# gildas-lormeau/zlib-streams-ts

Hardware: NVIDIA B200
Metric: deflate_input_GBps (higher is better)
Workload: dtype u8

## Files before the change

### zlib-streams-ts_b200/csrc/zs_lz77.cu

```cuda
#include <cstdio>
#include <cstdlib>

#include "zs_common.cuh"

namespace {

#ifndef ZS_SEARCH_WARPS
#define ZS_SEARCH_WARPS 30
#endif
#ifndef ZS_HASH_BITS
#define ZS_HASH_BITS 14
#endif
#ifndef ZS_LZ_PREV_POS
#define ZS_LZ_PREV_DELTA 1
#endif
constexpr int kSearchWarps = ZS_SEARCH_WARPS;
constexpr int kWarpParse = kSearchWarps;
constexpr int kWarpInsert = kSearchWarps + 1;
constexpr int kThreads = 32 * (kSearchWarps + 2);
constexpr int kStep = 32 * kSearchWarps;
constexpr unsigned kMaxDist = 32768u - 2u * kStep;
constexpr unsigned kNoPrev = 0xffffu;
constexpr unsigned kSymLimit = 16383u;
constexpr unsigned kTooFar = 4096u;
constexpr unsigned kHashBits = ZS_HASH_BITS;
constexpr unsigned kRing = 65536;
constexpr unsigned kRingGuard = 288;
constexpr unsigned pow2_at_least(unsigned v) { unsigned r = 1; while (r < v) r <<= 1; return r; }
constexpr unsigned kResRing = pow2_at_least(4 * kStep + 64);
constexpr unsigned kMjRing = pow2_at_least(3 * kStep + 64);
constexpr unsigned kPbRing = pow2_at_least(2 * kSearchWarps + 4);
constexpr unsigned kMaxSegChunks = 256;

struct LevelCfg { int lazy_fn, good, lazy, nice, chain; };
constexpr LevelCfg kLevels[10] = {
    {0, 0, 0, 0, 0},      {0, 4, 4, 8, 4},      {0, 4, 5, 16, 8},      {0, 4, 6, 32, 32},
    {1, 4, 4, 16, 16},    {1, 8, 16, 32, 32},   {1, 8, 16, 128, 128},  {1, 8, 32, 128, 256},
    {1, 32, 128, 258, 1024}, {1, 32, 258, 258, 4096}};
__host__ __device__ constexpr LevelCfg level_cfg(int level) { return kLevels[level]; }

constexpr uint32_t PREP_HAS_PRED = 1u << 21, PREP_LAST = 1u << 22, PREP_VALID = 1u << 23;

struct Smem {
    uint8_t ring[kRing + kRingGuard];
    uint16_t head[1 << kHashBits];
    uint16_t prev[32768];
    uint32_t prep[3 * kStep];
    uint16_t oldh[2 * kStep];
    uint2 pb[kPbRing];
    uint32_t res[kResRing];
    uint2 mj[kMjRing];
    uint32_t bnd[kMaxSegChunks + 1];
    uint32_t seg;
    uint32_t claim[2];
    alignas(8) uint64_t stage_bar;
};
static_assert(sizeof(Smem) <= 227 * 1024, "shared memory budget");

struct LzArgs {
    const uint8_t* buf;
    uint64_t org;
    uint64_t valid_lo;
    uint64_t data_end;
    const uint64_t* in_off;
    uint32_t n_chunks, seg_chunks, n_seg, max_bpc;
    uint32_t n_big, seg_small;
    LevelCfg cfg;
    int strategy;
    int cross;
    uint32_t* sym;
    uint32_t* chunk_nblk;
    uint32_t* blk_desc;
    uint32_t* seg_counter;
    unsigned stop_after, stop_active;
};

#ifdef ZS_LZ_PROF
__device__ unsigned long long g_prof[16];
#define PROF_T(i) if (lane == 0) atomicAdd(&g_prof[i], (unsigned long long)(clock64() - t_begin))
#else
#define PROF_T(i)
#endif

__device__ __forceinline__ unsigned res_slot(uint32_t q) { return q & (kResRing - 1u); }
__device__ __forceinline__ unsigned mj_slot(uint32_t q) { return q & (kMjRing - 1u); }

__device__ __forceinline__ uint32_t win32(const Smem& S, uint64_t pos) {
    const unsigned idx = (unsigned)pos & (kRing - 1u);
    const unsigned al = idx & ~3u;
    const uint32_t lo = *reinterpret_cast<const uint32_t*>(S.ring + al);
    const uint32_t hi = *reinterpret_cast<const uint32_t*>(S.ring + al + 4);
    return __funnelshift_r(lo, hi, (idx & 3u) * 8u);
}

__device__ __forceinline__ void stage_window(Smem& S, const LzArgs& a, uint64_t from, uint64_t to, unsigned tid, unsigned nthr) {
    const uint64_t safe16 = (a.data_end + 15) & ~15ull;
    for (uint64_t pos = from + 16ull * tid; pos < to; pos += 16ull * nthr) {
        uint4 v = make_uint4(0, 0, 0, 0);
        if (pos < safe16) v = __ldg(reinterpret_cast<const uint4*>(a.buf + pos));
        const unsigned idx = (unsigned)pos & (kRing - 1u);
        *reinterpret_cast<uint4*>(S.ring + idx) = v;
        if (idx < kRingGuard) *reinterpret_cast<uint4*>(S.ring + kRing + idx) = v;
    }
}

#ifndef ZS_LZ_NO_BULK
#define ZS_LZ_BULK 1
#endif
__device__ __forceinline__ unsigned smem_addr(const void* p) { return (unsigned)__cvta_generic_to_shared(p); }
__device__ __forceinline__ void mbar_init(uint64_t* bar, unsigned count) {
    asm volatile("mbarrier.init.shared::cta.b64 [%0], %1;" ::"r"(smem_addr(bar)), "r"(count) : "memory");
    asm volatile("fence.mbarrier_init.release.cluster;" ::: "memory");
}
__device__ __forceinline__ void mbar_expect_tx(uint64_t* bar, unsigned bytes) {
    asm volatile("mbarrier.arrive.expect_tx.shared::cta.b64 _, [%0], %1;" ::"r"(smem_addr(bar)), "r"(bytes) : "memory");
}
__device__ __forceinline__ void mbar_wait(uint64_t* bar, unsigned parity) {
    asm volatile(
        "{\n"
        ".reg .pred p;\n"
        "ZS_MBAR_WAIT:\n"
        "mbarrier.try_wait.parity.shared::cta.b64 p, [%0], %1;\n"
        "@p bra ZS_MBAR_DONE;\n"
        "bra ZS_MBAR_WAIT;\n"
        "ZS_MBAR_DONE:\n"
        "}\n" ::"r"(smem_addr(bar)), "r"(parity) : "memory");
}
__device__ __forceinline__ void bulk_g2s(void* dst, const void* src, unsigned bytes, uint64_t* bar) {
    asm volatile("cp.async.bulk.shared::cluster.global.mbarrier::complete_tx::bytes [%0], [%1], %2, [%3];" ::"r"(smem_addr(dst)),
                 "l"(src), "r"(bytes), "r"(smem_addr(bar))
                 : "memory");
}
__device__ __forceinline__ unsigned bulk_stage(Smem& S, const uint8_t* buf, uint64_t from, uint64_t to) {
    unsigned total = 0;
    while (from < to) {
        const unsigned idx = (unsigned)from & (kRing - 1u);
        unsigned nb = (unsigned)(to - from);
        if (idx + nb > kRing) nb = kRing - idx;
#ifdef ZS_DEBUG_HOOKS
        if (idx + nb > kRing || (nb & 15u) || (idx & 15u) || ((uintptr_t)(buf + from) & 15u)) { printf("[lz77 bulk] bad copy idx %u nb %u\n", idx, nb); __trap(); }
#endif
        bulk_g2s(S.ring + idx, buf + from, nb, &S.stage_bar);
        total += nb;
        if (idx < kRingGuard) {
            const unsigned g = idx + nb < kRingGuard ? nb : kRingGuard - idx;
#ifdef ZS_DEBUG_HOOKS
            if (idx + g > kRingGuard || (g & 15u)) { printf("[lz77 bulk] bad guard copy idx %u g %u\n", idx, g); __trap(); }
#endif
            bulk_g2s(S.ring + kRing + idx, buf + from, g, &S.stage_bar);
            total += g;
        }
        from += nb;
    }
    return total;
}

__device__ __forceinline__ unsigned hash3(uint32_t w) { return ((w & 0xffffffu) * 0x9E3779B1u) >> (32 - kHashBits); }

struct RangeCtx {
    uint32_t cb;
    uint32_t n;
    uint32_t pre;
    uint32_t tail;
    uint32_t q_data;
    uint32_t nc;
    int cross;
    unsigned min_len;
};

__device__ __forceinline__ uint32_t prep_batch(const Smem& S, const RangeCtx& c, uint32_t q0, uint32_t limit) {
    const unsigned lane = zs_lane();
    const uint32_t q = q0 + lane;
    const bool valid = q < limit && q + 2 < c.tail;
    unsigned h = 0;
    if (valid) h = hash3(win32(S, c.cb + q));
#ifndef ZS_PREP_MATCH_ANY
    unsigned peers = __ballot_sync(ZS_FULL_MASK, valid);
#pragma unroll
    for (int bit = 0; bit < (int)kHashBits; ++bit) {
        const bool one = (h >> bit) & 1u;
        const unsigned bal = __ballot_sync(ZS_FULL_MASK, one);
        peers &= one ? bal : ~bal;
    }
#else
    const unsigned peers = __match_any_sync(ZS_FULL_MASK, valid ? h : 0x10000u + lane);
#endif
    if (!valid) return 0u;
    const unsigned lower = peers & zs_lanemask_lt();
    uint32_t w = h | PREP_VALID;
    if (lower) w |= PREP_HAS_PRED | ((31u - __clz(lower)) << 16);
    if ((peers >> lane) == 1u) w |= PREP_LAST;
    return w;
}

__device__ __forceinline__ void head_exchange(Smem& S, uint32_t p16, uint32_t w, uint16_t* oldh) {
    const unsigned h = w & 0x7fffu;
    unsigned old = 0;
    if ((w & PREP_VALID) && !(w & PREP_HAS_PRED)) old = S.head[h];
    if (w & PREP_LAST) S.head[h] = (uint16_t)(p16 + zs_lane());
    oldh[zs_lane()] = (uint16_t)old;
    __syncwarp();
}
__device__ __forceinline__ void link_batch(Smem& S, const RangeCtx& c, uint32_t q0, uint32_t w, unsigned old) {
    if (w & PREP_VALID) {
        const uint32_t q = q0 + zs_lane();
        const unsigned p16 = (c.cb + q) & 0xffffu;
#ifdef ZS_LZ_PREV_DELTA
        unsigned hop = kNoPrev;
        if (w & PREP_HAS_PRED) {
            hop = zs_lane() - ((w >> 16) & 31u);
        } else {
            const unsigned delta = (p16 - old) & 0xffffu;
            if (delta != 0 && delta <= kMaxDist && delta <= q + c.pre) hop = delta;
        }
        S.prev[p16 & 32767u] = (uint16_t)hop;
#else
        unsigned pred = p16;
        if (w & PREP_HAS_PRED) {
            pred = (c.cb + q0 + ((w >> 16) & 31u)) & 0xffffu;
        } else {
            const unsigned delta = (p16 - old) & 0xffffu;
            if (delta != 0 && delta <= kMaxDist && delta <= q + c.pre) pred = (p16 - delta) & 0xffffu;
        }
        S.prev[p16 & 32767u] = (uint16_t)pred;
#endif
    }
}

#ifdef ZS_LZ_PREV_DELTA
__device__ __forceinline__ bool chain_hop(const Smem& S, unsigned& ci, unsigned& dist, unsigned max_back, unsigned& delta) {
    delta = S.prev[ci & 32767u];
    dist += delta;
    if (dist > max_back) return false;
    ci = (ci - delta) & (kRing - 1u);
    return true;
}
#else
__device__ __forceinline__ bool chain_hop(const Smem& S, unsigned& ci, unsigned& dist, unsigned max_back, unsigned& delta) {
    delta = (ci - S.prev[ci & 32767u]) & 0xffffu;
    if (delta == 0) return false;
    dist += delta;
    if (dist > max_back) return false;
    ci = (ci - delta) & (kRing - 1u);
    return true;
}
#endif

__device__ __forceinline__ uint32_t ring32(const Smem& S, unsigned idx) {
    idx &= kRing - 1u;
    const unsigned al = idx & ~3u;
    const uint32_t lo = *reinterpret_cast<const uint32_t*>(S.ring + al);
    const uint32_t hi = *reinterpret_cast<const uint32_t*>(S.ring + al + 4);
    return __funnelshift_r(lo, hi, (idx & 3u) * 8u);
}
__device__ __forceinline__ unsigned first_diff_byte(uint32_t x) { return (unsigned)(__ffs((int)x) - 1) >> 3; }

__device__ __forceinline__ uint2 ring64(const Smem& S, unsigned idx) {
    idx &= kRing - 1u;
    const unsigned al = idx & ~3u, sh = (idx & 3u) * 8u;
    const uint32_t w0 = *reinterpret_cast<const uint32_t*>(S.ring + al);
    const uint32_t w1 = *reinterpret_cast<const uint32_t*>(S.ring + al + 4);
    const uint32_t w2 = *reinterpret_cast<const uint32_t*>(S.ring + al + 8);
    return make_uint2(__funnelshift_r(w0, w1, sh), __funnelshift_r(w1, w2, sh));
}
__device__ __forceinline__ unsigned extend_match(const Smem& S, unsigned ci, unsigned pi, unsigned len, unsigned max_len) {
    unsigned aa = ((ci + len) & (kRing - 1u)) & ~3u, ab = ((pi + len) & (kRing - 1u)) & ~3u;
    const unsigned sa = ((ci + len) & 3u) * 8u, sb = ((pi + len) & 3u) * 8u;
    uint32_t a0 = *reinterpret_cast<const uint32_t*>(S.ring + aa);
    uint32_t b0 = *reinterpret_cast<const uint32_t*>(S.ring + ab);
    while (len < max_len) {
        const uint32_t a1 = *reinterpret_cast<const uint32_t*>(S.ring + aa + 4);
        const uint32_t a2 = *reinterpret_cast<const uint32_t*>(S.ring + aa + 8);
        const uint32_t b1 = *reinterpret_cast<const uint32_t*>(S.ring + ab + 4);
        const uint32_t b2 = *reinterpret_cast<const uint32_t*>(S.ring + ab + 8);
        const uint32_t yl = __funnelshift_r(a0, a1, sa) ^ __funnelshift_r(b0, b1, sb);
        const uint32_t yh = __funnelshift_r(a1, a2, sa) ^ __funnelshift_r(b1, b2, sb);
        if (yl | yh) return len + (yl ? first_diff_byte(yl) : 4u + first_diff_byte(yh));
        a0 = a2; b0 = b2;
        aa += 8; ab += 8;
        len += 8;
    }
    return len;
}
__device__ __forceinline__ unsigned match_length(const Smem& S, unsigned ci, unsigned pi, uint32_t pw0, uint32_t pw1, unsigned max_len) {
    const uint2 cw = ring64(S, ci);
    const uint32_t x0 = cw.x ^ pw0, x1 = cw.y ^ pw1;
    if (x0) return first_diff_byte(x0);
    if (x1) return 4u + first_diff_byte(x1);
    return extend_match(S, ci, pi, 8u, max_len);
}

constexpr unsigned kDenseHop = 8;
constexpr int kInteriorChain = 16;
template <int kMode, int kLevel>
__device__ __forceinline__ uint32_t search_position(const Smem& S, const LevelCfg& cfg, const RangeCtx& c, uint32_t q,
                                                    uint32_t cs, uint32_t ce) {
    static_assert(kMode == 0 || kMode == 2, "levels 4-9 go through search_lazy_endwin");
    const uint32_t room = ce - q;
    const unsigned max_len = room < 258u ? room : 258u;
    const unsigned pi = (c.cb + q) & (kRing - 1u);
    const uint2 pw = ring64(S, pi);
    const uint32_t pw0 = pw.x, pw1 = pw.y;
    const uint32_t lit = (pw0 & 0xffu) << 24;
    if (max_len < 3) return lit;
    if (kMode == 2) {
        const uint32_t back = c.cross ? q + c.pre : q - cs;
        if (back == 0) return lit;
        const uint32_t pat = (uint32_t)S.ring[(pi - 1u) & (kRing - 1u)] * 0x01010101u;
        unsigned len = 0;
        while (len < max_len) {
            const uint32_t x = ring32(S, pi + len) ^ pat;
            if (x) { len += first_diff_byte(x); break; }
            len += 4;
        }
        if (len > max_len) len = max_len;
        return len >= 3 ? (lit | (len << 15) | 1u) : lit;
    }
    const unsigned nice = (unsigned)cfg.nice < max_len ? (unsigned)cfg.nice : max_len;
    const uint32_t back = c.cross ? q + c.pre : q - cs;
    const unsigned max_back = back < kMaxDist ? back : kMaxDist;
    unsigned best_len = 2, best_dist = 0, best_ci = pi;
    unsigned ci = pi, dist = 0;
    if constexpr (kLevel != 0 && level_cfg(kLevel).nice <= 8) {
        bool alive = true;
        unsigned delta = S.prev[ci & 32767u];
#pragma unroll
        for (int round = 0; round < level_cfg(kLevel).chain; ++round) {
            dist += delta;
            alive = alive && dist <= max_back;
            ci = (ci - delta) & (kRing - 1u);
            const unsigned li = alive ? ci : pi;
            const uint2 cw = ring64(S, li);
            if (round + 1 < level_cfg(kLevel).chain) delta = S.prev[li & 32767u];
            const uint32_t x0 = cw.x ^ pw0, x1 = cw.y ^ pw1;
            const uint32_t xw = x0 ? x0 : x1;
            unsigned len = ((x0 ? 0u : 32u) + __popc((xw - 1u) & ~xw)) >> 3;
            if (len > max_len) len = max_len;
            if (alive && len > best_len) {
                best_len = len;
                best_dist = dist;
                best_ci = ci;
            }
            alive = alive && len < nice;
        }
    } else
    for (int chain = cfg.chain; chain > 0; --chain) {
        unsigned delta;
        if (!chain_hop(S, ci, dist, max_back, delta)) break;
        uint32_t x = ring32(S, ci) ^ pw0;
        if ((x & 0xffffffu) != 0) continue;
        unsigned len;
        if (x) {
            len = 3;
        } else {
            x = ring32(S, ci + 4) ^ pw1;
            if (x) {
                len = 4 + first_diff_byte(x);
            } else {
                len = 8;
                if (nice > 8u) len = extend_match(S, ci, pi, 8u, nice);
            }
        }
        if (len > max_len) len = max_len;
        if (len > best_len) {
            best_len = len;
            best_dist = dist;
            if (len >= nice) { best_ci = ci; break; }
        }
    }
    if (best_len >= nice) {
        best_len = extend_match(S, best_ci, pi, nice & ~7u, max_len);
        if (best_len > max_len) best_len = max_len;
    }
    if (best_len < c.min_len) return lit;
    if (best_len == 3 && best_dist > kTooFar) return lit;
    return lit | (best_len << 15) | best_dist;
}

struct StopCfg { unsigned after, active; };

__device__ __forceinline__ uint32_t search_lazy_endwin(const Smem& S, const LevelCfg& cfg, const StopCfg stop, const RangeCtx& c,
                                                       uint32_t q, uint32_t cs, uint32_t ce, bool live) {
    const uint32_t room = live ? ce - q : 0u;
    const unsigned max_len = room < 258u ? room : 258u;
    const unsigned pi = (c.cb + q) & (kRing - 1u);
    uint2 pw = make_uint2(0, 0);
    if (live) pw = ring64(S, pi);
    const uint32_t lit = (pw.x & 0xffu) << 24;
    const unsigned nice = (unsigned)cfg.nice < max_len ? (unsigned)cfg.nice : max_len;
    const uint32_t back = c.cross ? q + c.pre : q - cs;
    const unsigned max_back = back < kMaxDist ? back : kMaxDist;
    unsigned best_len = 2, best_dist = 0;
    unsigned ci = pi, dist = 0;
    unsigned woff = 0;
    uint32_t wown = pw.x, wmask = 0xffffffu;
    int chain = (live && max_len >= 3) ? cfg.chain : 0;
    for (unsigned it = 0;; ++it) {
        const unsigned walking = __ballot_sync(ZS_FULL_MASK, chain > 0);
        if (walking == 0) break;
        if (it >= stop.after && (unsigned)__popc(walking) <= stop.active) break;
        if (chain > 0) {
            do {
                unsigned delta;
                if (!chain_hop(S, ci, dist, max_back, delta)) { chain = 0; break; }
                if ((ring32(S, ci + woff) ^ wown) & wmask) {
                    if (delta <= kDenseHop && best_len >= 3) {
                        const uint2 cw = ring64(S, ci);
                        const uint32_t x0 = cw.x ^ pw.x, x1 = cw.y ^ pw.y;
                        const unsigned m = x0 ? first_diff_byte(x0) : x1 ? 4u + first_diff_byte(x1) : 8u;
                        if (m >= (best_len < 8u ? best_len : 8u)) chain -= chain >> 2;
                    }
                    break;
                }
                unsigned len = match_length(S, ci, pi, pw.x, pw.y, max_len);
                if (len > max_len) len = max_len;
                if (len > best_len) {
                    if (best_len < (unsigned)cfg.good && len >= (unsigned)cfg.good) {
                        const bool interior = S.ring[(ci - 1u) & (kRing - 1u)] == S.ring[(pi - 1u) & (kRing - 1u)];
                        if (interior || delta <= kDenseHop) chain >>= 2;
                        if (interior && chain > kInteriorChain) chain = kInteriorChain;
                    }
                    best_len = len;
                    best_dist = dist;
                    if (len >= nice) { chain = 0; break; }
                    woff = len - 3u; wmask = 0xffffffffu;
                    wown = ring32(S, pi + woff);
                } else if (len == best_len && delta <= kDenseHop) {
                    chain -= chain >> 2;
                }
            } while (0);
            --chain;
        }
    }
    if (best_len < c.min_len) return lit;
    if (best_len == 3 && best_dist > kTooFar) return lit;
    return lit | (best_len << 15) | best_dist;
}

constexpr unsigned MJ_MATCH = 1u << 9;
__device__ __forceinline__ unsigned mj_exit(unsigned y) { return y & 0x1ffu; }
__device__ __forceinline__ unsigned mj_count(unsigned y) { return (y >> 10) & 0x3fu; }
__device__ __forceinline__ unsigned mj_pair_exit(unsigned y) { return ((y >> 16) & 0x1ffu) + 32u; }
__device__ __forceinline__ unsigned mj_pair_count(unsigned y) { return y >> 25; }

template <int kMode>
__device__ __forceinline__ void resolve_one(const Smem& S, const LevelCfg& cfg, uint32_t n, uint32_t q0, unsigned& M,
                                            unsigned& J, bool& is_match) {
    const unsigned lane = zs_lane();
    const uint32_t q = q0 + lane;
    const uint32_t r = q < n ? S.res[res_slot(q)] : 0u;
    const unsigned L = (r >> 15) & 0x1ffu;
    unsigned Ln = __shfl_down_sync(ZS_FULL_MASK, L, 1);
    if (lane == 31) Ln = (q + 1 < n) ? ((S.res[res_slot(q + 1)] >> 15) & 0x1ffu) : 0u;
    const bool deferred = kMode == 1 && L >= 3 && L < (unsigned)cfg.lazy && Ln > L;
    is_match = L >= 3 && !deferred;
    J = q < n ? lane + (is_match ? L : 1u) : 32u;
    M = q < n ? 1u << lane : 0u;
#pragma unroll
    for (int round = 0; round < 5; ++round) {
        const unsigned src = J < 32 ? J : lane;
        const unsigned Mj = __shfl_sync(ZS_FULL_MASK, M, src);
        const unsigned Jj = __shfl_sync(ZS_FULL_MASK, J, src);
        if (J < 32) { M |= Mj; J = Jj; }
    }
}

template <int kMode>
__device__ __forceinline__ void resolve_pair(Smem& S, const LevelCfg& cfg, uint32_t n, uint32_t q0) {
    const unsigned lane = zs_lane();
    unsigned Ma, Ja, Mb, Jb;
    bool ma, mb;
    resolve_one<kMode>(S, cfg, n, q0, Ma, Ja, ma);
    resolve_one<kMode>(S, cfg, n, q0 + 32, Mb, Jb, mb);
    const unsigned ca = __popc(Ma), cb = __popc(Mb);
    const unsigned xa = Ja - 32u;
    const unsigned src = xa < 32u ? xa : lane;
    const unsigned jb = __shfl_sync(ZS_FULL_MASK, Jb, src), cbx = __shfl_sync(ZS_FULL_MASK, cb, src);
    const unsigned pair_exit = xa < 32u ? 32u + jb : Ja;
    const unsigned pair_cnt = xa < 32u ? ca + cbx : ca;
    const unsigned pe = pair_exit >= 32u ? pair_exit - 32u : 0u;
    if (q0 + lane < n)
        S.mj[mj_slot(q0 + lane)] = make_uint2(Ma, Ja | (ma ? MJ_MATCH : 0u) | (ca << 10) | (pe << 16) | (pair_cnt << 25));
    if (q0 + 32 + lane < n)
        S.mj[mj_slot(q0 + 32 + lane)] = make_uint2(Mb, Jb | (mb ? MJ_MATCH : 0u) | (cb << 10));
}

struct ParseState {
    uint32_t ppos;
    uint32_t skip;
    uint32_t nsym;
    uint32_t blk;
    uint32_t blk_sym0;
    uint32_t blk_pos0;
    uint32_t jc;
    uint32_t cstart;
    uint32_t nb;
};

__device__ __forceinline__ void close_block(const LzArgs& a, const RangeCtx& rc, ParseState& ps, uint32_t c0, uint32_t pos_end) {
    if (ps.blk < a.max_bpc && zs_lane() == 0) {
        uint32_t* d = a.blk_desc + ((uint64_t)(c0 + ps.jc) * a.max_bpc + ps.blk) * 4;
        d[0] = ps.blk_sym0 - (ps.cstart - rc.q_data);
        d[1] = ps.nsym - ps.blk_sym0;
        d[2] = ps.blk_pos0 - ps.cstart;
        d[3] = pos_end - ps.blk_pos0;
    }
    ps.blk++;
    ps.blk_sym0 = ps.nsym;
    ps.blk_pos0 = pos_end;
}

__device__ __forceinline__ void close_chunk(const Smem& S, const LzArgs& a, const RangeCtx& rc, ParseState& ps, uint32_t c0) {
    close_block(a, rc, ps, c0, ps.nb);
    if (zs_lane() == 0) a.chunk_nblk[c0 + ps.jc] = ps.blk < a.max_bpc ? ps.blk : a.max_bpc;
    ps.jc++;
    ps.cstart = ps.nb;
    ps.nb = ps.jc < rc.nc ? S.bnd[ps.jc + 1] : 0xffffffffu;
    ps.blk = 0;
}

__device__ __forceinline__ unsigned below(unsigned b) { return b >= 32u ? 0xffffffffu : (1u << b) - 1u; }

constexpr int kParseGroup = 16;
template <bool kBoundary>
__device__ __forceinline__ void parse_group(Smem& S, const LzArgs& a, const RangeCtx& rc, ParseState& ps, uint32_t c0,
                                            uint32_t qb, int np) {
    const unsigned lane = zs_lane();
    const uint32_t n = rc.n;
    unsigned ya[kParseGroup], yb[kParseGroup];
#pragma unroll
    for (int u = 0; u < kParseGroup; ++u) {
        const uint32_t q = qb + 64u * u + lane;
        ya[u] = (u < np && q < n) ? S.mj[mj_slot(q)].y : (32u | (32u << 16));
        yb[u] = (u < np && q + 32 < n) ? S.mj[mj_slot(q + 32)].y : 32u;
    }
#pragma unroll
    for (int u = 0; u < kParseGroup; ++u) {
        if (u < np) {
            const uint32_t q0 = qb + 64u * u;
            unsigned entry = 64u;
            const uint32_t first_sym = ps.nsym;
            if (ps.skip >= 64) {
                ps.skip -= 64;
            } else {
                unsigned s = ps.skip;
                entry = s;
                while (kBoundary && ps.nb < q0 + 64u) {
                    const unsigned b = ps.nb - q0;
                    unsigned c;
                    if (b <= s) {
                        c = 0;
                    } else if (s < 32u) {
                        const uint2 m = S.mj[mj_slot(q0 + s)];
                        c = __popc(m.x & below(b));
                        if (b > 32u) {
                            const unsigned xa = mj_exit(m.y) - 32u;
                            if (xa < b - 32u) c += __popc(S.mj[mj_slot(q0 + 32u + xa)].x & below(b - 32u));
                        }
                    } else {
                        c = __popc(S.mj[mj_slot(q0 + s)].x & below(b - 32u));
                    }
                    if (ps.nsym - ps.blk_sym0 + c > kSymLimit) close_block(a, rc, ps, c0, q0 + s);
                    ps.nsym += c;
                    close_chunk(S, a, rc, ps, c0);
                    s = b;
                }
                const unsigned wa = __shfl_sync(ZS_FULL_MASK, ya[u], s & 31u);
                const unsigned wb = __shfl_sync(ZS_FULL_MASK, yb[u], s & 31u);
                unsigned cnt, exit_rel;
                if (s < 32) { cnt = mj_pair_count(wa); exit_rel = mj_pair_exit(wa); }
                else { cnt = mj_count(wb); exit_rel = 32u + mj_exit(wb); }
                if (ps.nsym - ps.blk_sym0 + cnt > kSymLimit) close_block(a, rc, ps, c0, q0 + s);
                ps.nsym += cnt;
                ps.skip = exit_rel >= 64u ? exit_rel - 64u : 0u;
                while (kBoundary && ps.nb <= q0 + exit_rel) close_chunk(S, a, rc, ps, c0);
            }
            if (lane == 0) S.pb[(q0 >> 6) & (kPbRing - 1u)] = make_uint2(entry, first_sym);
        }
    }
}

__device__ __forceinline__ void emit_batch(const Smem& S, const LzArgs& a, uint64_t sym_base, uint32_t n, uint32_t q0) {
    const unsigned lane = zs_lane();
    const uint2 e = S.pb[(q0 >> 6) & (kPbRing - 1u)];
    if (e.x >= 64u) return;
    unsigned entry, first = e.y;
    if (!(q0 & 32u)) {
        if (e.x >= 32u) return;
        entry = e.x;
    } else if (e.x >= 32u) {
        entry = e.x - 32u;
    } else {
        const unsigned ya = S.mj[mj_slot(q0 - 32u + e.x)].y;
        const unsigned xa = mj_exit(ya) - 32u;
        if (xa >= 32u) return;
        entry = xa;
        first += mj_count(ya);
    }
    if (q0 + entry >= n) return;
    const unsigned visited = S.mj[mj_slot(q0 + entry)].x;
    if (((visited >> lane) & 1u) && q0 + lane < n) {
        const uint32_t q = q0 + lane;
        const uint32_t r = S.res[res_slot(q)];
        const bool is_match = (S.mj[mj_slot(q)].y & MJ_MATCH) != 0;
        a.sym[sym_base + first + __popc(visited & zs_lanemask_lt())] =
            is_match ? (((r & 0x7fffu) << 16) | ((r >> 15) & 0x1ffu)) : (r >> 24);
    }
}

__device__ __forceinline__ uint32_t resolved_frontier(uint32_t searched, uint32_t n) {
    if (searched >= n) return n;
    return searched >= 64 ? (searched - 1) & ~63u : 0;
}

template <int kMode, int kLevel>
__global__ void __launch_bounds__(kThreads, 1) lz77_kernel(LzArgs a) {
    static_assert(kLevel == 0 || (kMode == 0 && kLevel <= 3), "only the greedy levels are specialised");
    extern __shared__ __align__(16) unsigned char smem_raw[];
    Smem& S = *reinterpret_cast<Smem*>(smem_raw);
    const unsigned wid = threadIdx.x >> 5, lane = zs_lane();
    LevelCfg cfg = a.cfg;
    if constexpr (kLevel != 0) {
        constexpr LevelCfg row = level_cfg(kLevel);
        cfg = row;
    }
    const StopCfg stop = {a.stop_after, a.stop_active};
    (void)stop;

#ifdef ZS_LZ_BULK
    if (threadIdx.x == 0) mbar_init(&S.stage_bar, 1);
#endif
    for (;;) {
        if (threadIdx.x == 0) S.seg = atomicAdd(a.seg_counter, 1u);
        __syncthreads();
        const uint32_t seg = S.seg;
        if (seg >= a.n_seg) break;
        const bool big = seg < a.n_big;
        const uint32_t c0 = big ? seg * a.seg_chunks : a.n_big * a.seg_chunks + (seg - a.n_big) * a.seg_small;
        const uint32_t sc = big ? a.seg_chunks : a.seg_small;
        const uint32_t c1 = (c0 + sc < a.n_chunks) ? c0 + sc : a.n_chunks;

        const uint32_t nc = c1 - c0;

        if (threadIdx.x == 0) S.claim[0] = 0;
        {
            uint4* z = reinterpret_cast<uint4*>(S.head);
            const unsigned nz = (sizeof(S.head) + sizeof(S.prev)) / sizeof(uint4);
#ifdef ZS_LZ_PREV_DELTA
            const unsigned nh = sizeof(S.head) / sizeof(uint4);
            for (unsigned i = threadIdx.x; i < nz; i += kThreads) {
                const unsigned v = i < nh ? 0u : 0xffffffffu;
                z[i] = make_uint4(v, v, v, v);
            }
#else
            for (unsigned i = threadIdx.x; i < nz; i += kThreads) z[i] = make_uint4(0, 0, 0, 0);
#endif
        }
        const uint64_t off0 = a.in_off[c0];
        const uint64_t seg_start = a.org + off0;
        const uint64_t seg_end = a.org + a.in_off[c1];
        uint64_t prime0 = seg_start;
        if (a.cross) {
            prime0 = seg_start > a.valid_lo + 32768 ? seg_start - 32768 : a.valid_lo;
            prime0 = (prime0 + 31) & ~31ull;
            if (prime0 > seg_start) prime0 = seg_start;
        }
        RangeCtx rc;
        rc.cb = (uint32_t)prime0;
        rc.n = (uint32_t)(seg_end - prime0);
        rc.q_data = (uint32_t)(seg_start - prime0);
        rc.nc = nc;
        rc.cross = a.cross;
        rc.min_len = (kMode == 1 && a.strategy == ZS_STRATEGY_FILTERED) ? 6u : 3u;
        {
            const uint64_t pre = a.cross ? prime0 - a.valid_lo : 0;
            rc.pre = pre < kMaxDist ? (uint32_t)pre : kMaxDist;
            const uint64_t tail = a.data_end - prime0;
            rc.tail = tail < 0xffffffffull ? (uint32_t)tail : 0xffffffffu;
        }
        for (unsigned j = threadIdx.x; j <= nc; j += kThreads) S.bnd[j] = (uint32_t)(a.in_off[c0 + j] - off0) + rc.q_data;
        const uint64_t base16 = prime0 & ~15ull;
        const uint32_t p0lo = (uint32_t)prime0 & 15u;
        const uint32_t safe_rel = [&] {
            const uint64_t d = ((a.data_end + 15) & ~15ull) - base16;
            return d < 0xfffffff0ull ? (uint32_t)d : 0xfffffff0u;
        }();
        stage_window(S, a, base16, base16 + ((p0lo + 2u * kStep + kRingGuard + 15u) & ~15u), threadIdx.x, kThreads);
        __syncthreads();

        const uint32_t n = rc.n;
        const uint32_t nsteps = (n + kStep - 1) / kStep;
        const uint32_t n_iter = nsteps + 6;
        const uint32_t nwait = (nsteps + 1u) & ~1u;
        (void)nwait;
        const uint32_t qd64 = rc.q_data & ~63u;
        ParseState ps;
        ps.ppos = qd64; ps.skip = rc.q_data - qd64; ps.nsym = 0; ps.blk = 0; ps.blk_sym0 = 0; ps.blk_pos0 = rc.q_data;
        ps.jc = 0; ps.cstart = rc.q_data; ps.nb = S.bnd[1];
        if (wid == kWarpParse)
            while (ps.nb <= rc.q_data) close_chunk(S, a, rc, ps, c0);
        unsigned js = 0;
        uint32_t cs_w = rc.q_data, ce_w = S.bnd[1];
        uint32_t q_prep = 0;
        unsigned s_prep = 0;
        uint32_t searched = 0;
        uint32_t r0 = qd64, r1 = qd64, r2 = qd64, r3 = qd64;

        for (uint32_t k = 0; k < n_iter; ++k) {
#ifdef ZS_LZ_PROF
            const long long t_begin = clock64();
#endif
            r3 = r2; r2 = r1; r1 = r0;
            r0 = resolved_frontier(searched, n);
            if (r0 < qd64) r0 = qd64;
            const unsigned s_ins = s_prep == 0 ? 2u : s_prep - 1u;
            const unsigned s_link = s_ins == 0 ? 2u : s_ins - 1u;
            if (wid == kWarpInsert) {
                const uint32_t stage_from = (p0lo + q_prep + 2u * kStep + kRingGuard + 15u) & ~15u;
                const uint32_t stage_to = k < nsteps ? (p0lo + q_prep + 3u * kStep + kRingGuard + 15u) & ~15u : stage_from;
#ifdef ZS_LZ_BULK
                const uint32_t bulk_to = stage_to < safe_rel ? stage_to : safe_rel;
                if (k < nwait && lane == 0) {
                    unsigned total = 0;
                    if (stage_from < bulk_to) {
                        asm volatile("fence.proxy.async.shared::cta;" ::: "memory");
                        const unsigned i0 = ((uint32_t)base16 + stage_from) & (kRing - 1u), nb = bulk_to - stage_from;
                        total = nb;
                        if (i0 < kRingGuard) total += (i0 + nb < kRingGuard ? nb : kRingGuard - i0);
                        if (i0 + nb > kRing) total += (i0 + nb - kRing < kRingGuard ? i0 + nb - kRing : kRingGuard);
                    }
                    mbar_expect_tx(&S.stage_bar, total);
                    if (total) bulk_stage(S, a.buf, base16 + stage_from, base16 + bulk_to);
                }
#else
                constexpr int kStageVec = (kStep + 16 + 511) / 512;
                uint4 sv[kStageVec];
#pragma unroll
                for (int v = 0; v < kStageVec; ++v) {
                    const uint32_t pos = stage_from + 16u * (lane + 32 * v);
                    sv[v] = make_uint4(0, 0, 0, 0);
                    if (pos < stage_to && pos < safe_rel) sv[v] = __ldg(reinterpret_cast<const uint4*>(a.buf + base16 + pos));
                }
#endif
                if (k >= 1 && k - 1 < nsteps) {
                    const uint32_t p16 = rc.cb + q_prep - kStep;
                    const uint32_t* pw = S.prep + s_ins * kStep;
                    uint16_t* oh = S.oldh + ((k - 1) & 1u) * kStep;
#pragma unroll 8
                    for (int u = 0; u < kSearchWarps; ++u) head_exchange(S, p16 + 32u * u, pw[32 * u + lane], oh + 32 * u);
                }
#ifdef ZS_LZ_BULK
                if (stage_to > safe_rel) {
                    for (uint32_t pos = (stage_from > safe_rel ? stage_from : safe_rel) + 16u * lane; pos < stage_to; pos += 512u) {
                        const unsigned idx = ((uint32_t)base16 + pos) & (kRing - 1u);
                        *reinterpret_cast<uint4*>(S.ring + idx) = make_uint4(0, 0, 0, 0);
                        if (idx < kRingGuard) *reinterpret_cast<uint4*>(S.ring + kRing + idx) = make_uint4(0, 0, 0, 0);
                    }
                }
#ifdef ZS_LZ_BULK_DEBUG
                if (k < nwait) {
                    unsigned tries = 0, ok = 0;
                    while (!ok && tries < 200000u) {
                        asm volatile("{\n.reg .pred p;\nmbarrier.try_wait.parity.shared::cta.b64 p, [%1], %2;\nselp.u32 %0, 1, 0, p;\n}\n"
                                     : "=r"(ok) : "r"(smem_addr(&S.stage_bar)), "r"(k & 1u) : "memory");
                        ++tries;
                    }
                    if (!ok && lane == 0)
                        printf("[lz77 bulk] wait timed out: cta %u seg %u k %u of %u from %u to %u bulk_to %u safe %u p0lo %u base16 %llu\n",
                               blockIdx.x, seg, k, nsteps, stage_from, stage_to, bulk_to, safe_rel, p0lo, (unsigned long long)base16);
                }
#else
                if (k < nwait) mbar_wait(&S.stage_bar, k & 1u);
#endif
#else
#pragma unroll
                for (int v = 0; v < kStageVec; ++v) {
                    const uint32_t pos = stage_from + 16u * (lane + 32 * v);
                    if (pos < stage_to) {
                        const unsigned idx = ((uint32_t)base16 + pos) & (kRing - 1u);
                        *reinterpret_cast<uint4*>(S.ring + idx) = sv[v];
                        if (idx < kRingGuard) *reinterpret_cast<uint4*>(S.ring + kRing + idx) = sv[v];
                    }
                }
                if (stage_to > stage_from + 512u * kStageVec)
                    stage_window(S, a, base16 + stage_from + 512u * kStageVec, base16 + stage_to, lane, 32);
#endif
            } else if (wid == kWarpParse) {
                while (ps.ppos < r1) {
                    int np = (int)((r1 - ps.ppos + 63) / 64);
                    if (np > kParseGroup) np = kParseGroup;
                    if (ps.nb > ps.ppos + 64u * (unsigned)np + 258u) parse_group<false>(S, a, rc, ps, c0, ps.ppos, np);
                    else parse_group<true>(S, a, rc, ps, c0, ps.ppos, np);
                    ps.ppos += 64u * np;
                }
            } else {
                const unsigned i = wid * 32 + lane;
                if (k < nsteps) {
                    const uint32_t se = q_prep + kStep < n ? q_prep + kStep : n;
                    S.prep[s_prep * kStep + i] = prep_batch(S, rc, q_prep + 32u * wid, se);
                }
                if (k >= 2 && k - 2 < nsteps)
                    link_batch(S, rc, q_prep - 2u * kStep + 32u * wid, S.prep[s_link * kStep + i], S.oldh[(k & 1u) * kStep + i]);
                if (k >= 3 && k - 3 < nsteps) {
                    const uint32_t qw = q_prep - 3u * kStep + 32u * wid;
                    const uint32_t q = qw + lane;
                    if (qw + 32u > qd64 && qw < n) {
                        while (qw >= ce_w) { ++js; cs_w = ce_w; ce_w = S.bnd[js + 1]; }
                        uint32_t r = 0;
                        if constexpr (kMode == 1) {
                            const bool live = q >= rc.q_data && q < n;
                            uint32_t cs = cs_w, ce = ce_w;
                            if (live && q >= ce) {
                                unsigned jl = js;
                                do { ++jl; cs = ce; ce = S.bnd[jl + 1]; } while (q >= ce);
                            }
                            const uint32_t rr = search_lazy_endwin(S, cfg, stop, rc, q, cs, ce, live);
                            r = live ? rr : 0u;
                        } else
                        if (q >= rc.q_data && q < n) {
                            uint32_t cs = cs_w, ce = ce_w;
                            if (q >= ce) {
                                unsigned jl = js;
                                do { ++jl; cs = ce; ce = S.bnd[jl + 1]; } while (q >= ce);
                            }
                            r = search_position<kMode == 1 ? 0 : kMode, kLevel>(S, cfg, rc, q, cs, ce);
                        }
                        if (q < n) S.res[res_slot(q)] = r;
                    }
                }
                constexpr unsigned kHalf = kSearchWarps / 2;
#ifndef ZS_LZ_NO_CLAIM
                if constexpr (kMode == 1) {
                    const unsigned nr = r0 > r1 ? (r0 - r1 + 63u) >> 6 : 0u, ne = r2 > r3 ? (r2 - r3 + 63u) >> 6 : 0u;
                    if (threadIdx.x == 0) S.claim[(k + 1u) & 1u] = 0;
                    for (;;) {
                        unsigned item = 0;
                        if (lane == 0) item = atomicAdd(&S.claim[k & 1u], 1u);
                        item = __shfl_sync(ZS_FULL_MASK, item, 0);
                        if (item >= nr + ne) break;
                        if (item < nr) {
                            resolve_pair<kMode>(S, cfg, n, r1 + 64u * item);
                        } else {
                            const uint32_t q0 = r3 + 64u * (item - nr);
                            emit_batch(S, a, off0, n, q0);
                            if (q0 + 32 < r2) emit_batch(S, a, off0, n, q0 + 32);
                        }
                    }
                } else
#endif
                if (wid < kHalf) {
                    for (uint32_t q0 = r1 + 64u * wid; q0 < r0; q0 += 64u * kHalf) resolve_pair<kMode>(S, cfg, n, q0);
                } else {
                    for (uint32_t q0 = r3 + 64u * (wid - kHalf); q0 < r2; q0 += 64u * (kSearchWarps - kHalf)) {
                        emit_batch(S, a, off0, n, q0);
                        if (q0 + 32 < r2) emit_batch(S, a, off0, n, q0 + 32);
                    }
                }
            }
#ifdef ZS_LZ_PROF
            {
                const long long t_work = clock64() - t_begin;
                __syncwarp();
                if (lane == 0) {
                    const int role = wid == kWarpInsert ? 0 : wid == kWarpParse ? 1 : 2;
                    atomicAdd(&g_prof[role], (unsigned long long)t_work);
                    if (wid == 0) atomicAdd(&g_prof[4], 1ull);
                }
            }
#endif
            if (k >= 3) searched = searched + kStep < n ? searched + kStep : n;
            q_prep += kStep;
            s_prep = s_prep == 2 ? 0u : s_prep + 1u;
            __syncthreads();
#ifdef ZS_LZ_PROF
            if (threadIdx.x == 0) atomicAdd(&g_prof[3], (unsigned long long)(clock64() - t_begin));
#endif
        }
        if (wid == kWarpParse)
            while (ps.jc < nc) close_chunk(S, a, rc, ps, c0);
        __syncthreads();
    }
}

__global__ void plain_blocks_kernel(LzArgs a, uint32_t per_block, int with_symbols) {
    const uint32_t c = blockIdx.x * blockDim.x + threadIdx.x;
    if (c >= a.n_chunks) return;
    const uint32_t n = (uint32_t)(a.in_off[c + 1] - a.in_off[c]);
    uint32_t nb = (n + per_block - 1) / per_block;
    if (nb == 0) nb = 1;
    if (nb > a.max_bpc) nb = a.max_bpc;
    for (uint32_t j = 0; j < nb; j++) {
        uint32_t* d = a.blk_desc + ((uint64_t)c * a.max_bpc + j) * 4;
        const uint32_t b0 = j * per_block, len = n - b0 < per_block ? n - b0 : per_block;
        d[0] = with_symbols ? b0 : 0u;
        d[1] = with_symbols ? len : 0u;
        d[2] = b0;
        d[3] = len;
    }
    a.chunk_nblk[c] = nb;
}
__global__ void literal_symbols_kernel(const uint8_t* in, uint32_t* sym, uint64_t n) {
    for (uint64_t i = (uint64_t)blockIdx.x * blockDim.x + threadIdx.x; i < n; i += (uint64_t)gridDim.x * blockDim.x) sym[i] = in[i];
}

}

int zs_launch_lz77(zs_ctx* ctx, const zs_deflate_plan& p) {
    static bool attr_set[64] = {false};
    const int dev_slot = ctx->device >= 0 && ctx->device < 64 ? ctx->device : 0;
    using LzKernel = void (*)(LzArgs);
    static const LzKernel kGreedy[4] = {lz77_kernel<0, 0>, lz77_kernel<0, 1>, lz77_kernel<0, 2>, lz77_kernel<0, 3>};
    if (!attr_set[dev_slot] || ctx->device >= 64) {
        for (LzKernel k : kGreedy)
            ZS_CUDA_TRY(ctx, cudaFuncSetAttribute(k, cudaFuncAttributeMaxDynamicSharedMemorySize, (int)sizeof(Smem)));
        ZS_CUDA_TRY(ctx, cudaFuncSetAttribute(lz77_kernel<1, 0>, cudaFuncAttributeMaxDynamicSharedMemorySize, (int)sizeof(Smem)));
        ZS_CUDA_TRY(ctx, cudaFuncSetAttribute(lz77_kernel<2, 0>, cudaFuncAttributeMaxDynamicSharedMemorySize, (int)sizeof(Smem)));
        attr_set[dev_slot] = true;
    }
    LzArgs a;
    const uintptr_t first = reinterpret_cast<uintptr_t>(p.d_in) - p.history;
    const uintptr_t adj = first & 15u;
    a.buf = reinterpret_cast<const uint8_t*>(first - adj);
    a.valid_lo = adj;
    a.org = adj + p.history;
    a.data_end = a.org + p.in_len;
    a.in_off = p.d_in_off;
    a.n_chunks = p.n_chunks;
    a.max_bpc = p.max_bpc;
    a.cfg = kLevels[p.level];
    a.strategy = p.strategy;
    a.cross = (p.mode == ZS_MODE_STITCHED || (p.flags & ZS_FLAG_PRIME)) ? 1 : 0;
    uint32_t seg_chunks = 1;
    if (a.cross) {
        seg_chunks = p.n_chunks / (4u * (uint32_t)ctx->sm_count);
        if (seg_chunks < 1) seg_chunks = 1;
        if (seg_chunks > 16) seg_chunks = 16;
    } else {
        uint64_t waves = p.in_len / ((uint64_t)ctx->sm_count * (512u << 10));
        if (waves < 1) waves = 1;
        const uint64_t want = waves * (uint64_t)ctx->sm_count;
        uint64_t sc = (p.n_chunks + want - 1) / want;
        if (sc < 1) sc = 1;
        if (sc > kMaxSegChunks) sc = kMaxSegChunks;
        seg_chunks = (uint32_t)sc;
    }
    if (a.cross && p.seg_hint) seg_chunks = p.seg_hint < kMaxSegChunks ? p.seg_hint : kMaxSegChunks;
    a.seg_chunks = seg_chunks;
    a.seg_small = seg_chunks >= 4 ? seg_chunks / 4 : 1;
    a.n_big = (uint32_t)(((uint64_t)p.n_chunks * 3 / 4) / seg_chunks);
    {
        const uint32_t rest = p.n_chunks - a.n_big * seg_chunks;
        a.n_seg = a.n_big + (rest + a.seg_small - 1) / a.seg_small;
    }
    a.sym = p.d_sym;
    a.chunk_nblk = p.d_chunk_nblk;
    a.blk_desc = p.d_blk_desc;
    a.seg_counter = p.d_seg_counter;
    a.stop_after = 8;
    a.stop_active = 8;
    if (const char* e = getenv("ZS_LZ_STOP_AFTER")) a.stop_after = (unsigned)atoi(e);
    if (const char* e = getenv("ZS_LZ_STOP_ACTIVE")) a.stop_active = (unsigned)atoi(e);
    bool greedy_generic = false;
    if (const char* e = getenv("ZS_LZ_GREEDY_GENERIC")) greedy_generic = atoi(e) != 0;
#ifdef ZS_LZ_PROF
    if (const char* e = getenv("ZS_LZ_DEBUG"); e && (atoi(e) >> 8)) {
        a.cfg.chain = atoi(e) >> 8;
        greedy_generic = true;
    }
#endif
    if (p.level == 0 || p.strategy == ZS_STRATEGY_HUFFMAN_ONLY) {
        const bool stored = p.level == 0;
        ZS_KERNEL(ctx, "plain_blocks_kernel",
                  plain_blocks_kernel<<<(p.n_chunks + 127) / 128, 128, 0, ctx->stream>>>(a, stored ? 65535u : kSymLimit, stored ? 0 : 1));
        if (!stored && p.in_len)
            ZS_KERNEL(ctx, "literal_symbols_kernel",
                      literal_symbols_kernel<<<ctx->sm_count * 8, 256, 0, ctx->stream>>>(p.d_in, p.d_sym, p.in_len));
        return ZS_OK;
    }
    ZS_CUDA_TRY(ctx, cudaMemsetAsync(p.d_seg_counter, 0, sizeof(uint32_t), ctx->stream));
    unsigned grid = a.n_seg < (unsigned)ctx->sm_count ? a.n_seg : (unsigned)ctx->sm_count;
    if (grid == 0) return ZS_OK;
#ifdef ZS_DEBUG_HOOKS
    if (getenv("ZS_LZ_GRID")) { unsigned g = (unsigned)atoi(getenv("ZS_LZ_GRID")); if (g && g < grid) grid = g; }
#endif
#ifdef ZS_LZ_PROF
    unsigned long long zero[16] = {0};
    cudaMemcpyToSymbol(g_prof, zero, sizeof(zero));
#endif
    if (a.strategy == ZS_STRATEGY_RLE) {
        ZS_KERNEL(ctx, "lz77_kernel", lz77_kernel<2, 0><<<grid, kThreads, sizeof(Smem), ctx->stream>>>(a));
    } else if (p.level >= 4) {
        ZS_KERNEL(ctx, "lz77_kernel", lz77_kernel<1, 0><<<grid, kThreads, sizeof(Smem), ctx->stream>>>(a));
    } else {
        const LzKernel k = kGreedy[greedy_generic ? 0 : p.level];
        ZS_KERNEL(ctx, "lz77_kernel", k<<<grid, kThreads, sizeof(Smem), ctx->stream>>>(a));
    }
#ifdef ZS_LZ_PROF
    {
        unsigned long long pr[16];
        cudaStreamSynchronize(ctx->stream);
        cudaMemcpyFromSymbol(pr, g_prof, sizeof(pr));
        double st = pr[4] ? (double)pr[4] : 1.0;
        fprintf(stderr, "[lz77 prof] level %d steps %llu  cycles/step: insert %.0f parse %.0f wide(avg warp) %.0f step %.0f | insert: ldg-issued %.0f prep-loaded %.0f inserted %.0f | parse chain done %.0f\n",
                p.level, pr[4], pr[0] / st, pr[1] / st, pr[2] / st / kSearchWarps, pr[3] / st, pr[8] / st, pr[9] / st, pr[10] / st, pr[11] / st);
        fprintf(stderr, "[lz77 prof] chain-loop iterations: total %llu max %llu positions>100: %llu (last: best_len %llu at chunk offset %llu)\n",
                pr[12], pr[13], pr[14], pr[15] >> 32, pr[15] & 0xffffffffull);
    }
#endif
    return ZS_OK;
}
```

Before: 29.42.

## Streamline greedy parse fast path and simplify hash head exchange

The common-case parse group now walks match exits with one shared-memory load per 64-position batch. It no longer preloads 32 lanes of words and shuffles, and the symbol-limit check moves up into a stricter fast-path guard. Page-boundary bookkeeping is written once per group by the lanes, not by lane 0 per batch. The head exchange drops its predicate on the head read and fully unrolls the insert loop. Profiling also gains a max-warp timing counter. The serial parse chain becomes a dependent load chain with less shuffle overhead, which risks extra latency per step.

```diff
diff --git a/zlib-streams-ts_b200/csrc/zs_lz77.cu b/zlib-streams-ts_b200/csrc/zs_lz77.cu
--- a/zlib-streams-ts_b200/csrc/zs_lz77.cu
+++ b/zlib-streams-ts_b200/csrc/zs_lz77.cu
@@ -193,12 +193,11 @@
     return w;
 }
 
-__device__ __forceinline__ void head_exchange(Smem& S, uint32_t p16, uint32_t w, uint16_t* oldh) {
-    const unsigned h = w & 0x7fffu;
-    unsigned old = 0;
-    if ((w & PREP_VALID) && !(w & PREP_HAS_PRED)) old = S.head[h];
-    if (w & PREP_LAST) S.head[h] = (uint16_t)(p16 + zs_lane());
-    oldh[zs_lane()] = (uint16_t)old;
+__device__ __forceinline__ void head_exchange(Smem& S, uint32_t p, uint32_t w, uint16_t* oldh) {
+    const unsigned h = w & ((1u << kHashBits) - 1u);
+    const uint16_t old = S.head[h];
+    if (w & PREP_LAST) S.head[h] = (uint16_t)p;
+    oldh[zs_lane()] = old;
     __syncwarp();
 }
 __device__ __forceinline__ void link_batch(Smem& S, const RangeCtx& c, uint32_t q0, uint32_t w, unsigned old) {
@@ -522,62 +521,68 @@
 __device__ __forceinline__ unsigned below(unsigned b) { return b >= 32u ? 0xffffffffu : (1u << b) - 1u; }
 
 constexpr int kParseGroup = 16;
-template <bool kBoundary>
+template <bool kRare>
 __device__ __forceinline__ void parse_group(Smem& S, const LzArgs& a, const RangeCtx& rc, ParseState& ps, uint32_t c0,
                                             uint32_t qb, int np) {
     const unsigned lane = zs_lane();
     const uint32_t n = rc.n;
-    unsigned ya[kParseGroup], yb[kParseGroup];
-#pragma unroll
+    unsigned pb_entry = 64u, pb_sym = 0;
+    uint32_t pos = qb + ps.skip;
+    constexpr int kUnroll = kRare ? 1 : kParseGroup;
+#pragma unroll kUnroll
     for (int u = 0; u < kParseGroup; ++u) {
-        const uint32_t q = qb + 64u * u + lane;
-        ya[u] = (u < np && q < n) ? S.mj[mj_slot(q)].y : (32u | (32u << 16));
-        yb[u] = (u < np && q + 32 < n) ? S.mj[mj_slot(q + 32)].y : 32u;
-    }
-#pragma unroll
-    for (int u = 0; u < kParseGroup; ++u) {
-        if (u < np) {
-            const uint32_t q0 = qb + 64u * u;
-            unsigned entry = 64u;
-            const uint32_t first_sym = ps.nsym;
-            if (ps.skip >= 64) {
-                ps.skip -= 64;
-            } else {
-                unsigned s = ps.skip;
-                entry = s;
-                while (kBoundary && ps.nb < q0 + 64u) {
-                    const unsigned b = ps.nb - q0;
-                    unsigned c;
-                    if (b <= s) {
-                        c = 0;
-                    } else if (s < 32u) {
-                        const uint2 m = S.mj[mj_slot(q0 + s)];
-                        c = __popc(m.x & below(b));
-                        if (b > 32u) {
-                            const unsigned xa = mj_exit(m.y) - 32u;
-                            if (xa < b - 32u) c += __popc(S.mj[mj_slot(q0 + 32u + xa)].x & below(b - 32u));
-                        }
-                    } else {
-                        c = __popc(S.mj[mj_slot(q0 + s)].x & below(b - 32u));
+        if (u >= np) break;
+        const uint32_t q0 = qb + 64u * u;
+        const uint32_t first_sym = ps.nsym;
+        unsigned entry = 64u;
+        if constexpr (!kRare) {
+            const bool hop = pos < q0 + 64u, first = pos < q0 + 32u;
+            const unsigned y = S.mj[mj_slot(pos)].y;
+            const unsigned cnt = first ? mj_pair_count(y) : mj_count(y);
+            const unsigned e = (y >> (first ? 16u : 0u)) & 0x1ffu;
+            ps.nsym += hop ? cnt : 0u;
+            entry = hop ? pos - q0 : 64u;
+            if (hop) pos = q0 + 32u + e;
+        } else if (ps.skip >= 64) {
+            ps.skip -= 64;
+        } else {
+            unsigned s = ps.skip;
+            entry = s;
+            while (ps.nb < q0 + 64u) {
+                const unsigned b = ps.nb - q0;
+                unsigned c;
+                if (b <= s) {
+                    c = 0;
+                } else if (s < 32u) {
+                    const uint2 m = S.mj[mj_slot(q0 + s)];
+                    c = __popc(m.x & below(b));
+                    if (b > 32u) {
+                        const unsigned xa = mj_exit(m.y) - 32u;
+                        if (xa < b - 32u) c += __popc(S.mj[mj_slot(q0 + 32u + xa)].x & below(b - 32u));
                     }
-                    if (ps.nsym - ps.blk_sym0 + c > kSymLimit) close_block(a, rc, ps, c0, q0 + s);
-                    ps.nsym += c;
-                    close_chunk(S, a, rc, ps, c0);
-                    s = b;
-                }
-                const unsigned wa = __shfl_sync(ZS_FULL_MASK, ya[u], s & 31u);
-                const unsigned wb = __shfl_sync(ZS_FULL_MASK, yb[u], s & 31u);
-                unsigned cnt, exit_rel;
-                if (s < 32) { cnt = mj_pair_count(wa); exit_rel = mj_pair_exit(wa); }
-                else { cnt = mj_count(wb); exit_rel = 32u + mj_exit(wb); }
-                if (ps.nsym - ps.blk_sym0 + cnt > kSymLimit) close_block(a, rc, ps, c0, q0 + s);
-                ps.nsym += cnt;
-                ps.skip = exit_rel >= 64u ? exit_rel - 64u : 0u;
-                while (kBoundary && ps.nb <= q0 + exit_rel) close_chunk(S, a, rc, ps, c0);
+                } else {
+                    c = __popc(S.mj[mj_slot(q0 + s)].x & below(b - 32u));
+                }
+                if (ps.nsym - ps.blk_sym0 + c > kSymLimit) close_block(a, rc, ps, c0, q0 + s);
+                ps.nsym += c;
+                close_chunk(S, a, rc, ps, c0);
+                s = b;
             }
-            if (lane == 0) S.pb[(q0 >> 6) & (kPbRing - 1u)] = make_uint2(entry, first_sym);
-        }
-    }
+            unsigned cnt = 0, exit_rel = 64u;
+            if (q0 + s < n) {
+                const unsigned y = S.mj[mj_slot(q0 + s)].y;
+                if (s < 32) { cnt = mj_pair_count(y); exit_rel = mj_pair_exit(y); }
+                else { cnt = mj_count(y); exit_rel = 32u + mj_exit(y); }
+            }
+            if (ps.nsym - ps.blk_sym0 + cnt > kSymLimit) close_block(a, rc, ps, c0, q0 + s);
+            ps.nsym += cnt;
+            ps.skip = exit_rel >= 64u ? exit_rel - 64u : 0u;
+            while (ps.nb <= q0 + exit_rel) close_chunk(S, a, rc, ps, c0);
+        }
+        if (lane == (unsigned)u) { pb_entry = entry; pb_sym = first_sym; }
+    }
+    if constexpr (!kRare) ps.skip = pos - (qb + 64u * np);
+    if (lane < (unsigned)np) S.pb[((qb >> 6) + lane) & (kPbRing - 1u)] = make_uint2(pb_entry, pb_sym);
 }
 
 __device__ __forceinline__ void emit_batch(const Smem& S, const LzArgs& a, uint64_t sym_base, uint32_t n, uint32_t q0) {
@@ -629,6 +634,10 @@
 
 #ifdef ZS_LZ_BULK
     if (threadIdx.x == 0) mbar_init(&S.stage_bar, 1);
+#endif
+#ifdef ZS_LZ_PROF
+    __shared__ unsigned long long prof_wmax[2];
+    if (threadIdx.x < 2) prof_wmax[threadIdx.x] = 0;
 #endif
     for (;;) {
         if (threadIdx.x == 0) S.seg = atomicAdd(a.seg_counter, 1u);
@@ -743,11 +752,11 @@
                 }
 #endif
                 if (k >= 1 && k - 1 < nsteps) {
-                    const uint32_t p16 = rc.cb + q_prep - kStep;
-                    const uint32_t* pw = S.prep + s_ins * kStep;
+                    const uint32_t p = rc.cb + q_prep - kStep + lane;
+                    const uint32_t* pw = S.prep + s_ins * kStep + lane;
                     uint16_t* oh = S.oldh + ((k - 1) & 1u) * kStep;
-#pragma unroll 8
-                    for (int u = 0; u < kSearchWarps; ++u) head_exchange(S, p16 + 32u * u, pw[32 * u + lane], oh + 32 * u);
+#pragma unroll
+                    for (int u = 0; u < kSearchWarps; ++u) head_exchange(S, p + 32u * u, pw[32 * u], oh + 32 * u);
                 }
 #ifdef ZS_LZ_BULK
                 if (stage_to > safe_rel) {
@@ -789,8 +798,10 @@
                 while (ps.ppos < r1) {
                     int np = (int)((r1 - ps.ppos + 63) / 64);
                     if (np > kParseGroup) np = kParseGroup;
-                    if (ps.nb > ps.ppos + 64u * (unsigned)np + 258u) parse_group<false>(S, a, rc, ps, c0, ps.ppos, np);
-                    else parse_group<true>(S, a, rc, ps, c0, ps.ppos, np);
+                    if (ps.nb > ps.ppos + 64u * (unsigned)np + 258u && ps.nsym - ps.blk_sym0 + 64u * (unsigned)np <= kSymLimit)
+                        parse_group<false>(S, a, rc, ps, c0, ps.ppos, np);
+                    else
+                        parse_group<true>(S, a, rc, ps, c0, ps.ppos, np);
                     ps.ppos += 64u * np;
                 }
             } else {
@@ -864,6 +875,7 @@
                 if (lane == 0) {
                     const int role = wid == kWarpInsert ? 0 : wid == kWarpParse ? 1 : 2;
                     atomicAdd(&g_prof[role], (unsigned long long)t_work);
+                    if (role == 2) atomicMax(&prof_wmax[k & 1u], (unsigned long long)t_work);
                     if (wid == 0) atomicAdd(&g_prof[4], 1ull);
                 }
             }
@@ -873,7 +885,11 @@
             s_prep = s_prep == 2 ? 0u : s_prep + 1u;
             __syncthreads();
 #ifdef ZS_LZ_PROF
-            if (threadIdx.x == 0) atomicAdd(&g_prof[3], (unsigned long long)(clock64() - t_begin));
+            if (threadIdx.x == 0) {
+                atomicAdd(&g_prof[3], (unsigned long long)(clock64() - t_begin));
+                atomicAdd(&g_prof[5], prof_wmax[k & 1u]);
+                prof_wmax[k & 1u] = 0;
+            }
 #endif
         }
         if (wid == kWarpParse)
@@ -1001,8 +1017,8 @@
         cudaStreamSynchronize(ctx->stream);
         cudaMemcpyFromSymbol(pr, g_prof, sizeof(pr));
         double st = pr[4] ? (double)pr[4] : 1.0;
-        fprintf(stderr, "[lz77 prof] level %d steps %llu  cycles/step: insert %.0f parse %.0f wide(avg warp) %.0f step %.0f | insert: ldg-issued %.0f prep-loaded %.0f inserted %.0f | parse chain done %.0f\n",
-                p.level, pr[4], pr[0] / st, pr[1] / st, pr[2] / st / kSearchWarps, pr[3] / st, pr[8] / st, pr[9] / st, pr[10] / st, pr[11] / st);
+        fprintf(stderr, "[lz77 prof] level %d steps %llu  cycles/step: insert %.0f parse %.0f wide(avg warp) %.0f wide(max warp) %.0f step %.0f | insert: ldg-issued %.0f prep-loaded %.0f inserted %.0f | parse chain done %.0f\n",
+                p.level, pr[4], pr[0] / st, pr[1] / st, pr[2] / st / kSearchWarps, pr[5] / st, pr[3] / st, pr[8] / st, pr[9] / st, pr[10] / st, pr[11] / st);
         fprintf(stderr, "[lz77 prof] chain-loop iterations: total %llu max %llu positions>100: %llu (last: best_len %llu at chunk offset %llu)\n",
                 pr[12], pr[13], pr[14], pr[15] >> 32, pr[15] & 0xffffffffull);
     }
```

Result: faster. 34.67 (median of 6 runs) (+17.8%).
